# b4rtaz/distributed-llama

Hardware: AMD Instinct MI355X
Metric: decode tokens/s (Llama-3.1-8B Q40) (higher is better)
Workload: dtype f32-accum/int8-dot (Q40 weights, Q80 activations); 1 GPU; model=llama-3.1-8b, global_batch=1, seq_len=4096, prefill=32, parallelism=tp1, sync=q80, graph=True

## Files before the change

### dllama_amd/engine.py

```python

from __future__ import annotations

import time
from dataclasses import dataclass

import torch

from .tokenizer import Sampler


@dataclass
class GenStats:
    prefill_tokens: int = 0
    prefill_time: float = 0.0
    decode_tokens: int = 0
    decode_time: float = 0.0
    cached_tokens: int = 0

    @property
    def eval_tok_s(self) -> float:
        return self.prefill_tokens / self.prefill_time if self.prefill_time else 0.0

    @property
    def pred_tok_s(self) -> float:
# ... 100 lines not shown
            else:
                logits = self.decode_one(token)
                token = sampler.sample(logits)
            out.append(token)
            if on_token:
                on_token(token)
        self._sync_device()
        stats.decode_time = time.perf_counter() - t0
        stats.decode_tokens = len(out)
        return out, stats


class _Sequence:

    def __init__(self, prompt, max_tokens, sampler, on_token, stop_check):
        self.prompt = list(prompt)
        self.max_tokens = max_tokens
        self.sampler = sampler
        self.on_token = on_token
        self.stop_check = stop_check
        self.slot = None
        self.fed = 0
        self.pages = []
        self.registered = 0
        self.written = 0
        self.out: list[int] = []
        self.done = False
        self.stats = GenStats(prefill_tokens=len(self.prompt))
        self._t0 = None

    @property
    def tokens(self) -> list[int]:
        return self.out

    @property
    def prefilling(self) -> bool:
        return self.fed < len(self.prompt)


class BatchEngine:

    def __init__(self, model, tokenizer=None, n_batches: int = 32,
                 share_prefixes: bool = True):
        if not hasattr(model, "forward_rows"):
            raise ValueError("BatchEngine needs a model with forward_rows")
        self.model = model
        self.pool = None
        if getattr(model, "page_map", None) is not None:
            from .models.pages import PagePool
            self.pool = PagePool(model.kv_pages, model.page_size,
                                 share=share_prefixes)
            for slot in range(model.n_slots):
                model.clear_slot(slot)
        self.tokenizer = tokenizer
        self.n_batches = min(n_batches, getattr(model, "n_batches", n_batches))
        self.seq_len = model.cfg.seq_len
        self.free_slots = list(range(model.n_slots))
        self.waiting: list[_Sequence] = []
        self.running: list[_Sequence] = []
        self.last_step_rows: list[tuple] = []

    _coin = staticmethod(InferenceEngine._coin)

    def _on_device(self) -> bool:
        return (hasattr(self.model, "forward_rows_sample")
                and bool(getattr(self.model, "device_sampling", False)))

    def submit(self, prompt_tokens: list[int], max_tokens: int,
               sampler: Sampler | None = None, on_token=None,
               stop_check=None) -> _Sequence:
        if len(prompt_tokens) < 1:
            raise ValueError("empty prompt")
        if len(prompt_tokens) > self.seq_len:
            raise ValueError(
                f"prompt of {len(prompt_tokens)} tokens exceeds seq_len "
                f"{self.seq_len} (rebuild with a larger --max-seq-len / seq_len)")
        if self.pool is not None:
            need = self._pages_needed(len(prompt_tokens), max_tokens)
            if need > self.pool.n_pages:
                raise ValueError(
                    f"a request of {len(prompt_tokens)} prompt tokens and "
                    f"max_tokens {max_tokens} needs {need} KV pages, the pool "
                    f"has {self.pool.n_pages} (raise --kv-pages / kv_pages)")
        if sampler is None:
            sampler = Sampler(self.model.cfg.vocab_size, 0.0, 0.9, 12345)
        seq = _Sequence(prompt_tokens, max_tokens, sampler, on_token,
                        stop_check)
        self.waiting.append(seq)
        return seq

    @property
    def idle(self) -> bool:
        return not self.waiting and not self.running

    def _pages_needed(self, n_prompt: int, max_tokens: int) -> int:
        P = self.pool.page_size
        return -(-min(n_prompt + max_tokens, self.seq_len) // P)

    def _take_pages(self, seq: _Sequence) -> bool:
        pool = self.pool
        shared = pool.match(seq.prompt)
        need = self._pages_needed(len(seq.prompt), seq.max_tokens)
        new = pool.alloc(need - len(shared))
        if new is None:
            pool.release(shared)
            return False
# ... 128 lines not shown
```

### dllama_amd/models/hip_model.py

```python

from __future__ import annotations

import os

import numpy as np
import torch

from ..model_file import HIDDEN_ACT_GELU, ModelFile, ROPE_FALCON
from ..ops import hip_ops
from ..ops import reference as R
from ..ops.sampler import DeviceSampler
from ..parallel.comm import Comm, SingleComm
from ..quants import Q80, q40_to_planes
from .config import ModelConfig

QB = 32


class Linear:

    def __init__(self, qs: torch.Tensor, scales: torch.Tensor):
        self.qs = qs
        self.scales = scales
        self.d = qs.shape[-2]
# ... 71 lines not shown
        self.kv_pages = kv_pages
        self.page_size = page_size
        self.page_map = None
        self.page_table_sends = 0
        if kv_pages:
            from .rows import PageMap
            self.page_map = PageMap(n_slots, c.seq_len, kv_pages, page_size)
        self.comm = comm or SingleComm()
        self.tp_path = config.world > 1 or force_sync
        self.device = torch.device(device or "cuda")
        self.k = hip_ops()
        nb = 32
        if n_batches != 32:
            import warnings
            warnings.warn(
                f"HIP backend pins --n-batches to 32 (got {n_batches}): the "
                "prefill GEMM's MFMA fragment is 32 batch rows")
        self.n_batches = nb
        self.layers: list[dict] = []
        self.embedding = None
        self.final_norm = None
        self.wcls = None
        self._graph = None
        self._graph_pos = None
        self._graph_samples = False
        self._dev_sampler = None
        self.greedy_feedback = False
        self.skip_logits = False
        self._pf_graphs = {}
        self._pf_failed = False
        self.row_graphs = True
        self._row_graphs = {}
        self._row_graphs_failed = False
        self._rows_io = None
        self.kv_mul = c.n_heads0 // max(1, c.kv_dim0 // c.head_dim)
        self.rope_style = 1 if c.rope_type == ROPE_FALCON else 0
        self.fused_rope = self.rope_style == 0 and not c.is_qwen3
        self.row_bytes = c.dim + 2 * (c.dim // QB)
        self._read_options()
        self._alloc_buffers()

    def _read_options(self):
        env = os.environ

        def flag(name: str, default: str) -> bool:
            return env.get(name, default) == "1"

        self.attn_splits = int(env.get("DLLAMA_ATTN_SPLITS", "8"))
        self.fused_sync = flag("DLLAMA_FUSED_SYNC", "1")
        self.adaptive_thresh = int(env.get("DLLAMA_ADAPTIVE_SPLITS", "512"))
        if ("DLLAMA_ATTN_SPLITS" in env
                and "DLLAMA_ADAPTIVE_SPLITS" not in env):
            self.adaptive_thresh = 0
        self.fused_ffn = flag("DLLAMA_FUSED_FFN", "0")
        self.fused_moe = flag("DLLAMA_FUSED_MOE", "0")
        self.use_deferred = flag("DLLAMA_DEFERRED", "1")
        self.prefill_bf16 = flag("DLLAMA_PREFILL_BF16", "0")
        self.ksplit_resid = int(env.get("DLLAMA_KSPLIT_RESID", "0"))
        self.kv_f32 = flag("DLLAMA_KV_F32", "0")


    @classmethod
    def from_file(cls, m: ModelFile, config: ModelConfig, device=None,
                  comm: Comm | None = None, n_batches: int = 32,
                  force_sync: bool = False,
                  n_slots: int = 1, kv_pages: int = 0,
                  page_size: int = 64) -> "HipTransformer":
        from ..quants import Q40
        if m.header.weight_type != Q40:
            raise ValueError(
                "the MI355X HIP backend runs Q40 weights (the reference's "
                "shipped format); f32/q80 .m files run on the CPU backend "
                "(--gpu-index -1) or can be re-quantized with convert_hf.py")
        self = cls(config, device, comm, n_batches, force_sync, n_slots,
                   kv_pages, page_size)
        c, dev = config, self.device
        r, w = c.rank, c.world

        def lin(name, layer, d, n, expert=-1):
            e = m.entry(name, layer, expert)
            raw = m.slice_bytes(e, r, w)
            return Linear.from_blocks(raw, d, n, dev)

        def f32(name, layer=-1):
            return torch.from_numpy(np.array(m.f32(name, layer))).to(dev)

        def w13(l, expert=-1):
            return Linear.cat(lin("block_matmul_w1", l, c.ff_dim0, c.dim, expert),
                              lin("block_matmul_w3", l, c.ff_dim0, c.dim, expert))

        self.embedding = f32("embedding")
        self.final_norm = f32("final_norm")
        self.wcls = lin("final_matmul_logits", -1, c.vocab0, c.dim)
        for l in range(c.n_layers):
            lw = {
                "qkv": Linear.cat(lin("block_matmul_q", l, c.q_dim0, c.dim),
                                  lin("block_matmul_k", l, c.kv_dim0, c.dim),
                                  lin("block_matmul_v", l, c.kv_dim0, c.dim)),
                "wo": lin("block_matmul_wo", l, c.dim, c.q_dim0),
                "norm0": f32("block_norm_0", l),
                "norm1": f32("block_norm_1", l),
            }
            if c.is_moe:
                experts = range(c.n_experts)
                lw["gate"] = f32("block_moe_gate", l)
                lw["w13"] = Linear.stack([w13(l, e) for e in experts])
# ... 406 lines not shown
                           self.moe_idx[:ka], self.moe_out13, ka,
                           ssq_in=self.ssq[slot], eps=c.norm_eps)
        self._swiglu_q80(self.moe_out13, ka, self.moe_dq)
        k.q40_gemv_grouped(lw["w2"].qs, lw["w2"].scales, *self.moe_dq.triple(),
                           self.moe_idx[:ka], self.moe_y, 1)
        if self.tp_path:
            k.scale_merge_pack(self.moe_y, self.moe_wts,
                               self.sync_out[: self.row_bytes], 1, ka, c.dim)
            self._wire_exchange(1, self.ssq[slot + 1], wn)
        else:
            k.scale_merge_add_q(self.x[:1], self.moe_y, self.moe_wts,
                                self.ssq[slot + 1], wn, *self.xq.triple(),
                                1, ka)

    def _moe_ffn(self, B: int, NB: int, lw: dict, slot: int):
        c, k = self.cfg, self.k
        ka = c.n_active_experts
        S = NB * ka
        k.router_gemv(lw["gate"], self.t_norm, self.moe_router, NB)
        if c.ff_dim0 % 32 == 0 and ka <= 16 and self.fused_moe:
            wts, gate = self.moe_router[:NB], {"gate": True}
            k.q40_gemv_grouped_swiglu(lw["w13"].qs, lw["w13"].scales,
                                      *self.xq.triple(), *self.moe_dq.triple(),
                                      S, wts, ka)
            k.q40_gemv_grouped(lw["w2"].qs, lw["w2"].scales,
                               *self.moe_dq.triple(), self.moe_idx[:S],
                               self.moe_y, 1, router=wts, topk=ka, n_slots=S)
        else:
            wts, gate = self.moe_wts, {}
            k.moe_gate(self.moe_router[:NB], self.moe_idx, self.moe_wts, NB, ka)
            k.q40_gemv_grouped(lw["w13"].qs, lw["w13"].scales,
                               *self.xq.triple(), self.moe_idx[:S],
                               self.moe_out13, ka)
            self._swiglu_q80(self.moe_out13, S, self.moe_dq)
            k.q40_gemv_grouped(lw["w2"].qs, lw["w2"].scales,
                               *self.moe_dq.triple(), self.moe_idx[:S],
                               self.moe_y, 1)
        if not self.tp_path:
            k.scale_merge_add(self.x[:NB], self.moe_y, wts, self.ssq[slot],
                              NB, ka, **gate)
        else:
            k.scale_merge(self.partial[:NB], self.moe_y, wts, NB, ka, **gate)
            self._sync_partial(NB, slot)


    def forward(self, tokens: torch.Tensor, positions: torch.Tensor) -> torch.Tensor:
        B = tokens.shape[0]
        assert B <= self.n_batches
        p0 = self._first_position(positions, B)
        self.tokens[:B].copy_(tokens.to(self.device), non_blocking=True)
        if B == 1 and self._graph is not None:
            self._replay_decode(p0)
        else:
            g = None
            if B == self.n_batches and not self._pf_failed:
                g = (self._pf_graphs.get(self.skip_logits)
                     or self._capture_prefill_graph(self.skip_logits))
            self._step_at(B, p0, g)
        if self.tp_path:
            NBp = _pow2_batch(B)
            self.k.logits_concat(self.logits_full, self.logits_gather[NBp], B)
            return self.logits_full[:B]
        return self.logits0[:B]

    def _first_position(self, positions, B: int) -> int:
        self._rows_only()
        p0 = int(positions[0])
        if p0 + B > self.cfg.seq_len:
            raise ValueError(
                f"position {p0}+{B} exceeds seq_len {self.cfg.seq_len} "
                "(rebuild with a larger --max-seq-len / seq_len)")
        return p0

    def _step_at(self, B: int, p0: int, graph=None):
        self.pos.fill_(p0)
        self._graph_pos = None
        if graph is not None:
            graph.replay()
        else:
            self.forward_buffers(B)

    def _replay_decode(self, p0: int):
        sp = self._pick_splits(p0)
        if sp != self.attn_splits:
            self._set_attn_splits(sp)
        if p0 != self._graph_pos:
            self.pos.fill_(p0)
        self._graph.replay()
        self._graph_pos = p0 + 1


    def last_logits(self) -> torch.Tensor:
        if self.tp_path:
            return self.logits_gather[1].view(-1)[: self.cfg.vocab_size]
        return self.logits0[0]

    def _sampler(self) -> DeviceSampler:
        if self._dev_sampler is None:
            self._dev_sampler = DeviceSampler(
                self.cfg.vocab_size, self.device, params=self.sample_params,
                out=self.sample_out, k=self.k)
            self._step_host = torch.zeros(self.n_batches + 4,
                                          dtype=torch.int64).pin_memory()
        return self._dev_sampler

    def sample_row(self, row: torch.Tensor, coin, temperature: float,
                   topp: float):
        return self._sampler().sample(row, coin, temperature, topp)

    def forward_sample(self, tokens: torch.Tensor, positions: torch.Tensor,
                       coin, temperature: float, topp: float):
        assert tokens.shape[0] == 1
        p0 = self._first_position(positions, 1)
        smp, NB = self._sampler(), self.n_batches
        self._step_host[0] = int(tokens[0])
        smp.fill_params(self._step_host[NB:].view(torch.float64), coin,
                        temperature, topp)
        self._step_in.copy_(self._step_host, non_blocking=True)
        if self._graph is not None:
            self._replay_decode(p0)
            if not self._graph_samples:
                smp.launch(self.last_logits())
        else:
            self._step_at(1, p0)
            smp.launch(self.last_logits())
        return smp.read()


    def _rows_only(self):
        if self.page_map is not None:
            raise ValueError(
                "a paged model steps rows only (forward_rows); one sequence "
                "runs on the unpaged default")

    def _paged(self):
        if self.page_map is None:
            raise ValueError("the model has no paged KV cache (kv_pages=0)")
        return self.page_map

    def set_slot_pages(self, slot: int, pages, first: int = 0) -> None:
        self._paged().set_slot_pages(slot, pages, first)

    def clear_slot(self, slot: int) -> None:
        self._paged().clear_slot(slot)

    def _send_page_table(self):
        pm = self.page_map
        for slot in sorted(pm.dirty):
            self.page_table[slot].copy_(
                torch.tensor(pm.device_row(slot), dtype=torch.int32))
            self.page_table_sends += 1
        pm.dirty.clear()


    def _rows_buffers(self):
        if self._rows_io is None:
            NB, dev = self.n_batches, self.device
            self._rows_io = io = torch.zeros(6 * NB, dtype=torch.int64, device=dev)
            self.row_tokens = io[:NB]
            self.row_params = io[NB:5 * NB].view(torch.float64).view(NB, 4)
            self.rows = io[5 * NB:].view(torch.int32).view(NB, 2)
            if self.page_map is not None:
                self.row_addr = KVAddr("_paged", self.rows, self.page_table,
                                       self.page_size)
            else:
                self.row_addr = KVAddr("_rows", self.rows)
            self.rows_sample_out = torch.zeros(NB, 2, dtype=torch.int64,
                                               device=dev)
            self._rows_host = torch.zeros(6 * NB, dtype=torch.int64)
            if dev.type == "cuda":
                self._rows_host = self._rows_host.pin_memory()
            self._rows_copied = None
            self._rows_dev = []
            self._row_samplers = []
        return self._rows_io

# ... 20 lines not shown
            self.page_map.check(slots, positions)
            self._send_page_table()
            stride = self.page_map.pages_per_seq
        self._rows_buffers()
        if self._rows_copied is not None:
            self._rows_copied.synchronize()
        host = self._rows_host
        table = [(s * stride, p) for s, p in zip(slots, positions)]
        host[:NB] = 0
        host[:B] = torch.tensor(tokens, dtype=torch.int64)
        hp = host[NB:5 * NB].view(torch.float64).view(NB, 4)
        hp.zero_()
        if params is not None:
            hp[:B, :3] = torch.tensor(params, dtype=torch.float64)
        words = 5 * NB
        if self._rows_dev[:B] != table:
            ht = host[5 * NB:].view(torch.int32).view(NB, 2)
            ht.zero_()
            ht[:B] = torch.tensor(table, dtype=torch.int32)
            words = 6 * NB
            self._rows_dev = list(table)
        self._rows_io[:words].copy_(host[:words], non_blocking=True)
        if self.device.type == "cuda":
            self._rows_copied = torch.cuda.Event()
            self._rows_copied.record(torch.cuda.current_stream(self.device))
        return B, table, is_decode_step(slots)

    def _forward_rows_buffers(self, B: int):
        self._forward_explicit(B, self.row_addr)

    def _rows_step_and_sample(self, B: int):
        self._forward_rows_buffers(B)
        logits = self.rows_logits(B)
        for b in range(B):
            self._row_sampler(b).launch(logits[b])

    def _capture_rows_graph(self, B: int):
        try:
            for b in range(B):
                self._row_sampler(b)
            g = self._capture(lambda: self._rows_step_and_sample(B), warmups=2,
                              tail=lambda: self.k.rows_advance(self.rows, B))
            self._row_graphs[B] = g
            return g
        except Exception as e:
            import sys
            if self.comm.rank == 0:
                print(f"⚠️  row-step graph capture failed ({e}); "
                      "running eager (slower)", file=sys.stderr)
            self._row_graphs_failed = True
            return None

    def _run_rows(self, B: int, table, decode_only: bool, sample: bool):
        sp = self._pick_splits(max(p for _, p in table))
        if sp != self.attn_splits:
            self._set_attn_splits(sp)
        g = None
        if (decode_only and self.row_graphs and not self._row_graphs_failed
                and self.device.type == "cuda"):
            g = self._row_graphs.get(B) or self._capture_rows_graph(B)
        if g is not None:
            g.replay()
            self._rows_dev[:B] = [(base, p + 1) for base, p in table]
        elif sample:
            self._rows_step_and_sample(B)
        else:
            self._forward_rows_buffers(B)

    def forward_rows(self, tokens, slots, positions) -> torch.Tensor:
        B, table, decode_only = self._stage_rows(tokens, slots, positions)
        self._run_rows(B, table, decode_only, sample=False)
        return self.rows_logits(B)

    def forward_rows_sample(self, tokens, slots, positions, coins,
                            temperatures, topps) -> list:
        params = [(0.0 if c is None else float(c), float(t), float(p))
                  for c, t, p in zip(coins, temperatures, topps)]
        if len(params) != len(tokens):
            raise ValueError("one coin, temperature and topp per row")
        B, table, decode_only = self._stage_rows(tokens, slots, positions,
                                                 params)
        self._run_rows(B, table, decode_only, sample=True)
        return [None if status else token
                for token, status in self.rows_sample_out[:B].tolist()]


    def _pick_splits(self, pos: int) -> int:
        if not self.adaptive_thresh:
            return self.attn_splits
        if pos < self.adaptive_thresh:
            return 8
        return 16 if pos < 2048 else 32

    def _set_attn_splits(self, s: int):
        self.attn_splits = s
        self._alloc_attn_scratch()
        if self._graph is not None:
            pos_saved = int(self.pos.item())
            self.capture_decode_graph()
            self.pos.fill_(pos_saved)
            self._graph_pos = pos_saved
        self._pf_graphs.clear()
        self._row_graphs.clear()

    def _capture(self, body, warmups: int, tail=None):
        dev = self.device
        torch.cuda.synchronize(dev)
        s = torch.cuda.Stream(dev)
        s.wait_stream(torch.cuda.current_stream(dev))
        with torch.cuda.stream(s):
            for _ in range(warmups):
                body()
        torch.cuda.current_stream(dev).wait_stream(s)
        torch.cuda.synchronize(dev)
        g = torch.cuda.CUDAGraph()
        with torch.cuda.graph(g):
            body()
            if tail is not None:
                tail()
        return g

    def _capture_prefill_graph(self, skip_logits: bool):
        try:
            saved = self.skip_logits
            self.skip_logits = skip_logits
            g = self._capture(lambda: self.forward_buffers(self.n_batches),
                              warmups=1)
            self.skip_logits = saved
            self._pf_graphs[skip_logits] = g
            return g
        except Exception:
            self._pf_failed = True
            self.skip_logits = skip_logits
            return None

    def capture_decode_graph(self):
        self._rows_only()
        sample = bool(self.device_sampling)
        if sample:
            self._sampler()

        def step():
            self.forward_buffers(1)
            if sample:
                self._sampler().launch(self.last_logits())

        self._graph = self._capture(
            step, warmups=2, tail=lambda: self.k.pos_inc(self.pos, 1))
# ... 3 lines not shown
```

### dllama_amd/ops/csrc/attn.hip

```cpp

#include "dllama_common.h"

struct SeqRows {
    static constexpr bool kPaged = false;
    const int *pos;
    __device__ int position(int b) const { return pos[0] + b; }
    __device__ int64_t cache_base(int) const { return 0; }
    __device__ int64_t cache_row(int, int t) const { return t; }
};
struct TableRows {
    static constexpr bool kPaged = false;
    const int *rows;
    __device__ int position(int b) const { return rows[2 * b + 1]; }
    __device__ int64_t cache_base(int b) const { return rows[2 * b]; }
    __device__ int64_t cache_row(int b, int t) const {
        return (int64_t)rows[2 * b] + t;
    }
};
struct PagedRows {
    static constexpr bool kPaged = true;
    const int *rows;
    const int *pages;
    int shift;
    __device__ int position(int b) const { return rows[2 * b + 1]; }
    __device__ int64_t cache_base(int) const { return 0; }
    __device__ const int *seq_pages(int b) const { return pages + rows[2 * b]; }
    __device__ int64_t cache_row(int b, int t) const {
        return ((int64_t)seq_pages(b)[t >> shift] << shift)
             + (t & ((1 << shift) - 1));
    }
};

template <int VEC, typename KVT, bool FUSE = false, typename ROWS = SeqRows>
__global__ void k_attn_split(const float *__restrict__ q, int q_ld,
                             const KVT *__restrict__ kc_all,
                             const KVT *__restrict__ vc_all,
                             const ROWS rows,
                             int n_heads0, int kv_mul, int kv_dim0, float scale,
                             float *__restrict__ ml_scratch,
                             float *__restrict__ o_scratch,
                             int *__restrict__ counter,
                             float *__restrict__ y,
                             int8_t *__restrict__ zq,
                             float *__restrict__ zs,
                             float *__restrict__ zbs) {
    (void)counter; (void)y; (void)zq; (void)zs; (void)zbs;
    const int h0 = blockIdx.x;
    const int b = blockIdx.y;
    const int sp = blockIdx.z;
    const int S = gridDim.z;
    const int hd = VEC * WAVE;
    const int plen = rows.position(b) + 1;
    const KVT *kc = kc_all + rows.cache_base(b) * kv_dim0;
    const KVT *vc = vc_all + rows.cache_base(b) * kv_dim0;
    const int wave = ROWS::kPaged
        ? __builtin_amdgcn_readfirstlane(threadIdx.x / WAVE)
        : threadIdx.x / WAVE;
    const int lane = threadIdx.x % WAVE;
    const int kv_off = (h0 / kv_mul) * hd;

    const int VEC16 = VEC * 4;
    const int lane16 = lane & 15;
    const int group = lane >> 4;

    float qreg[VEC16];
    #pragma unroll
    for (int v = 0; v < VEC16; v++)
        qreg[v] = q[(int64_t)b * q_ld + h0 * hd + lane16 * VEC16 + v] * scale;

    float m = -1e30f, l = 0.0f, o[VEC];
    #pragma unroll
    for (int v = 0; v < VEC; v++) o[v] = 0.0f;

    const int stride = 16 * S;
    [[maybe_unused]] int pg[4];
    [[maybe_unused]] const int *seq_pages = nullptr;
    [[maybe_unused]] int pshift = 0;
    if constexpr (ROWS::kPaged) {
        seq_pages = rows.seq_pages(b);
        pshift = rows.shift;
        #pragma unroll
        for (int u = 0; u < 4; u++) {
            const int t = (sp * 4 + wave) * 4 + u * stride;
            pg[u] = t < plen ? seq_pages[t >> pshift] : 0;
        }
    }
    for (int tb0 = (sp * 4 + wave) * 4; tb0 < plen; tb0 += 4 * stride) {
        [[maybe_unused]] int64_t rb[4];
        if constexpr (ROWS::kPaged) {
            #pragma unroll
            for (int u = 0; u < 4; u++) {
                const int t = tb0 + u * stride;
                rb[u] = ((int64_t)pg[u] << pshift) + (t & ((1 << pshift) - 1));
            }
            #pragma unroll
            for (int u = 0; u < 4; u++) {
                const int t = tb0 + 4 * stride + u * stride;
                pg[u] = t < plen ? seq_pages[t >> pshift] : 0;
            }
// ... 14 lines not shown
        }
        float s16[16];
        float mn = m;
        #pragma unroll
        for (int u = 0; u < 4; u++) {
            #pragma unroll
            for (int gg = 0; gg < 4; gg++) {
                float v = __shfl(su[u], gg * 16, WAVE);
                if (tb0 + u * stride + gg >= plen) v = -1e30f;
                s16[4 * u + gg] = v;
                mn = fmaxf(mn, v);
            }
        }
        const float f = __expf(m - mn);
        float w16[16];
        float lsum = 0.0f;
        #pragma unroll
        for (int i = 0; i < 16; i++) {
            w16[i] = __expf(s16[i] - mn);
            lsum += w16[i];
        }
        l = l * f + lsum;
        #pragma unroll
        for (int v = 0; v < VEC; v++) o[v] *= f;
        #pragma unroll
        for (int u = 0; u < 4; u++) {
            #pragma unroll
            for (int gg = 0; gg < 4; gg++) {
                const int t = tb0 + u * stride + gg;
                if (t >= plen) continue;
                const int64_t vr = ROWS::kPaged ? rb[u] + gg : (int64_t)t;
                const KVT *vrow = vc + vr * kv_dim0 + kv_off + lane * VEC;
                #pragma unroll
                for (int v = 0; v < VEC; v++)
                    o[v] = fmaf(w16[4 * u + gg], kv_f(vrow[v]), o[v]);
            }
        }
        m = mn;
    }

    __shared__ float sm[4], sl[4];
    __shared__ float so[4][VEC * WAVE];
    if (lane == 0) { sm[wave] = m; sl[wave] = l; }
    __syncthreads();
    const float M = fmaxf(fmaxf(sm[0], sm[1]), fmaxf(sm[2], sm[3]));
    const float fw = __expf(m - M);
    #pragma unroll
    for (int v = 0; v < VEC; v++) so[wave][lane * VEC + v] = o[v] * fw;
    __syncthreads();
    const int64_t slot = ((int64_t)b * n_heads0 + h0) * S + sp;
    if (wave == 0) {
        const float L = sl[0] * __expf(sm[0] - M) + sl[1] * __expf(sm[1] - M)
                      + sl[2] * __expf(sm[2] - M) + sl[3] * __expf(sm[3] - M);
        if constexpr (FUSE) {
            const float invL = 1.0f / L;
            float vv[VEC];
            #pragma unroll
            for (int v = 0; v < VEC; v++) {
                const int i = lane * VEC + v;
                vv[v] = (so[0][i] + so[1][i] + so[2][i] + so[3][i]) * invL;
            }
            if constexpr (VEC == 2) {
                const float amax = group16_reduce_max(fmaxf(fabsf(vv[0]), fabsf(vv[1])));
                const float dd = amax / 127.0f;
                const float qinv = dd > 0.0f ? 1.0f / dd : 0.0f;
                const float q0 = rintf(vv[0] * qinv), q1 = rintf(vv[1] * qinv);
                const int64_t obase = ((int64_t)b * n_heads0 + h0) * hd + lane * 2;
                zq[obase] = (int8_t)q0;
                zq[obase + 1] = (int8_t)q1;
                const float bsum = group16_reduce_sum(q0 + q1);
                if ((lane & 15) == 0) {
                    const int blk = (h0 * hd + lane * 2) / QB;
                    zs[(int64_t)b * (n_heads0 * hd / QB) + blk] = dd;
                    zbs[(int64_t)b * (n_heads0 * hd / QB) + blk] = bsum;
                }
            } else {
                const Q80Lane c = q80_quant_group32(vv[0]);
                zq[((int64_t)b * n_heads0 + h0) * hd + lane] = (int8_t)c.qf;
                const float bsum = group32_reduce_sum(c.qf);
                if ((lane & 31) == 0) {
                    const int blk = (h0 * hd + lane) / QB;
                    zs[(int64_t)b * (n_heads0 * hd / QB) + blk] = c.d;
                    zbs[(int64_t)b * (n_heads0 * hd / QB) + blk] = bsum;
                }
            }
        } else {
            if (lane == 0) {
                ml_scratch[slot * 2] = M;
                ml_scratch[slot * 2 + 1] = L;
            }
            #pragma unroll
            for (int v = 0; v < VEC; v++) {
                const int i = lane * VEC + v;
                o_scratch[slot * hd + i] = so[0][i] + so[1][i] + so[2][i] + so[3][i];
            }
        }
    }

}

template <int VEC, typename KVT>
__global__ void k_attn_split_gqa(const float *__restrict__ q, int q_ld,
                                 const KVT *__restrict__ kc,
                                 const KVT *__restrict__ vc,
                                 const int *__restrict__ pos,
                                 int n_heads0, int kv_mul, int kv_dim0,
                                 float scale,
                                 float *__restrict__ ml_scratch,
                                 float *__restrict__ o_scratch) {
    const int kvh = blockIdx.x;
    const int b = blockIdx.y;
    const int sp = blockIdx.z;
    const int S = gridDim.z;
    const int hd = VEC * WAVE;
    const int plen = pos[0] + b + 1;
    const int wave = threadIdx.x / WAVE;
    const int lane = threadIdx.x % WAVE;
    const int h0 = kvh * kv_mul + wave;
    const int kv_off = kvh * hd;
    const int VEC16 = VEC * 4;
    const int lane16 = lane & 15;
    const int group = lane >> 4;

    float qreg[VEC16];
    #pragma unroll
    for (int v = 0; v < VEC16; v++)
        qreg[v] = q[(int64_t)b * q_ld + h0 * hd + lane16 * VEC16 + v] * scale;

    float m = -1e30f, l = 0.0f, o[VEC];
    #pragma unroll
    for (int v = 0; v < VEC; v++) o[v] = 0.0f;

    for (int tb0 = sp * 16; tb0 < plen; tb0 += 16 * S) {
        float su[4];
        #pragma unroll
        for (int u = 0; u < 4; u++) {
            const int tg = tb0 + u * 4 + group;
            float partial = 0.0f;
            if (tg < plen) {
                const KVT *krow = kc + (int64_t)tg * kv_dim0 + kv_off + lane16 * VEC16;
                #pragma unroll
                for (int v = 0; v < VEC16; v++)
                    partial = fmaf(qreg[v], kv_f(krow[v]), partial);
            }
            su[u] = group16_reduce_sum(partial);
        }
        float s16[16];
        float mn = m;
        #pragma unroll
        for (int u = 0; u < 4; u++) {
            #pragma unroll
            for (int gg = 0; gg < 4; gg++) {
// ... 267 lines not shown

void kv_append(torch::Tensor k, torch::Tensor v, torch::Tensor kc,
               torch::Tensor vc, torch::Tensor pos) {
    CHECK_CUDA(k);
    const int B = k.size(0);
    const int kv_dim0 = k.size(1);
    const dim3 grid(ceil_div(kv_dim0, 256), B);
    with_kv_ptrs(kc, vc, [&](auto *kcp, auto *vcp) {
        using KVT = std::remove_pointer_t<decltype(kcp)>;
        hipLaunchKernelGGL(k_kv_append<KVT>, grid, dim3(256), 0, cur_stream(),
                           k.data_ptr<float>(), v.data_ptr<float>(), kcp, vcp,
                           pos.data_ptr<int>(), kv_dim0);
    });
}

static TableRows table_rows(const torch::Tensor &rows, int64_t batch) {
    CHECK_CUDA(rows);
    TORCH_CHECK(rows.scalar_type() == at::kInt && rows.dim() == 2
                && rows.size(1) == 2 && rows.is_contiguous()
                && rows.size(0) >= batch,
                "row table must be a contiguous int32 [>= batch, 2]");
    return TableRows{rows.data_ptr<int>()};
}

static PagedRows paged_rows(const torch::Tensor &rows,
                            const torch::Tensor &page_table, int64_t page_size,
                            int64_t batch, const torch::Tensor &kc) {
    const TableRows t = table_rows(rows, batch);
    CHECK_CUDA(page_table);
    TORCH_CHECK(page_table.scalar_type() == at::kInt && page_table.dim() == 2
                && page_table.is_contiguous() && page_table.numel() > 0
                && page_table.device() == kc.device()
                && rows.device() == kc.device(),
                "page table must be a contiguous int32 [n_slots, "
                "pages_per_seq] on the cache's device");
    TORCH_CHECK(page_size >= 4 && page_size <= 256
                && (page_size & (page_size - 1)) == 0,
                "page_size must be a power of two in 4..256 (got ",
                page_size, ")");
    TORCH_CHECK(kc.size(0) % page_size == 0,
                "a paged cache holds whole pages: ", kc.size(0),
                " rows, page_size ", page_size);
    int shift = 0;
    while ((int64_t(1) << shift) < page_size) shift++;
    return PagedRows{t.rows, page_table.data_ptr<int>(), shift};
}

template <typename ROWS>
static void attn_launch(torch::Tensor &q, int64_t q_ld, torch::Tensor &kc,
                        torch::Tensor &vc, torch::Tensor &y, ROWS rows,
                        int64_t batch, int64_t n_heads0, int64_t kv_mul,
                        int64_t head_dim, int64_t splits,
                        torch::Tensor &ml_scratch, torch::Tensor &o_scratch,
                        int *counter, bool allow_variants,
                        c10::optional<torch::Tensor> &zq,
                        c10::optional<torch::Tensor> &zs,
                        c10::optional<torch::Tensor> &zbs) {
    CHECK_CUDA(q);
    const int kv_dim0 = kc.size(1);
    const float scale = 1.0f / sqrtf((float)head_dim);
    const dim3 grid(n_heads0, batch, splits);
    const dim3 cgrid(n_heads0, batch);
    const bool quant = zq.has_value();
    float *yp = quant ? nullptr : y.data_ptr<float>();
    int8_t *zqp = quant ? zq->data_ptr<int8_t>() : nullptr;
    float *zsp = quant ? zs->data_ptr<float>() : nullptr;
    float *zbsp = quant ? zbs->data_ptr<float>() : nullptr;
    static const bool env_gqa =
        std::getenv("DLLAMA_GQA_ATTN") && atoi(std::getenv("DLLAMA_GQA_ATTN")) == 1;
    const bool gqa = allow_variants && env_gqa && kv_mul > 1 && kv_mul <= 8
        && n_heads0 % kv_mul == 0 && splits > 1;
    const bool fused = allow_variants && !gqa && splits == 1 && quant;
    with_head_vec(head_dim, [&](auto vec_const) {
        constexpr int V = decltype(vec_const)::value;
        with_kv_ptrs(kc, vc, [&](auto *kcp, auto *vcp) {
            using KVT = std::remove_pointer_t<decltype(kcp)>;
            auto split = [&](auto fuse_const) {
                constexpr bool FUSE = decltype(fuse_const)::value;
                hipLaunchKernelGGL((k_attn_split<V, KVT, FUSE, ROWS>), grid,
                                   dim3(256), 0,
                                   cur_stream(), q.data_ptr<float>(), (int)q_ld,
                                   kcp, vcp, rows,
                                   (int)n_heads0, (int)kv_mul, kv_dim0, scale,
                                   ml_scratch.data_ptr<float>(),
                                   o_scratch.data_ptr<float>(),
                                   counter, nullptr,
                                   FUSE ? zqp : nullptr, FUSE ? zsp : nullptr,
                                   FUSE ? zbsp : nullptr);
            };
            if constexpr (std::is_same_v<ROWS, SeqRows>) {
                if (gqa) {
                    hipLaunchKernelGGL((k_attn_split_gqa<V, KVT>),
                                       dim3(n_heads0 / kv_mul, batch, splits),
                                       dim3(kv_mul * WAVE), 0,
                                       cur_stream(), q.data_ptr<float>(), (int)q_ld,
                                       kcp, vcp, rows.pos, (int)n_heads0,
                                       (int)kv_mul, kv_dim0, scale,
                                       ml_scratch.data_ptr<float>(),
                                       o_scratch.data_ptr<float>());
                    return;
                }
                if (fused) {
                    split(std::true_type{});
                    return;
                }
            }
            split(std::false_type{});
        });
        if (fused) return;
        auto combine = [&](auto quant_const) {
            hipLaunchKernelGGL((k_attn_combine<V, decltype(quant_const)::value>),
                               cgrid, dim3(V * WAVE), 0, cur_stream(),
                               ml_scratch.data_ptr<float>(),
                               o_scratch.data_ptr<float>(), yp, zqp, zsp, zbsp,
                               (int)n_heads0, (int)splits);
        };
        if (quant) combine(std::true_type{});
        else combine(std::false_type{});
    });
}

void attn(torch::Tensor q, int64_t q_ld, torch::Tensor kc, torch::Tensor vc,
          torch::Tensor y, torch::Tensor pos, int64_t batch, int64_t n_heads0,
          int64_t kv_mul, int64_t head_dim, int64_t splits,
          torch::Tensor ml_scratch, torch::Tensor o_scratch, torch::Tensor counter,
          c10::optional<torch::Tensor> zq = c10::nullopt,
          c10::optional<torch::Tensor> zs = c10::nullopt,
          c10::optional<torch::Tensor> zbs = c10::nullopt) {
    attn_launch(q, q_ld, kc, vc, y, SeqRows{pos.data_ptr<int>()}, batch,
                n_heads0, kv_mul, head_dim, splits, ml_scratch, o_scratch,
                counter.data_ptr<int>(), true, zq, zs, zbs);
}

void attn_rows(torch::Tensor q, int64_t q_ld, torch::Tensor kc, torch::Tensor vc,
               torch::Tensor y, torch::Tensor rows, int64_t batch,
               int64_t n_heads0, int64_t kv_mul, int64_t head_dim,
               int64_t splits, torch::Tensor ml_scratch, torch::Tensor o_scratch,
               c10::optional<torch::Tensor> zq = c10::nullopt,
               c10::optional<torch::Tensor> zs = c10::nullopt,
               c10::optional<torch::Tensor> zbs = c10::nullopt) {
    attn_launch(q, q_ld, kc, vc, y, table_rows(rows, batch), batch, n_heads0,
                kv_mul, head_dim, splits, ml_scratch, o_scratch, nullptr,
                false, zq, zs, zbs);
}

void attn_paged(torch::Tensor q, int64_t q_ld, torch::Tensor kc, torch::Tensor vc,
                torch::Tensor y, torch::Tensor rows, torch::Tensor page_table,
                int64_t page_size, int64_t batch, int64_t n_heads0,
                int64_t kv_mul, int64_t head_dim, int64_t splits,
                torch::Tensor ml_scratch, torch::Tensor o_scratch,
                c10::optional<torch::Tensor> zq = c10::nullopt,
                c10::optional<torch::Tensor> zs = c10::nullopt,
                c10::optional<torch::Tensor> zbs = c10::nullopt) {
    attn_launch(q, q_ld, kc, vc, y,
                paged_rows(rows, page_table, page_size, batch, kc), batch,
                n_heads0, kv_mul, head_dim, splits, ml_scratch, o_scratch,
                nullptr, false, zq, zs, zbs);
}

template <typename ROWS>
static void rope_kv_launch(torch::Tensor &qkv, int64_t ld, int64_t q_dim0,
                           int64_t kv_dim0, torch::Tensor &cache, ROWS rows,
                           torch::Tensor &kc, torch::Tensor &vc,
                           int64_t head_dim, int64_t style, int64_t batch) {
    CHECK_CUDA(qkv);
    const int total = (int)(q_dim0 / 2 + kv_dim0 / 2 + kv_dim0 / 4);
    const dim3 grid(ceil_div(total, 256), batch);
    with_kv_ptrs(kc, vc, [&](auto *kcp, auto *vcp) {
        using KVT = std::remove_pointer_t<decltype(kcp)>;
        auto *kern = style == 0 ? k_rope_kv<0, KVT, ROWS> : k_rope_kv<1, KVT, ROWS>;
        hipLaunchKernelGGL(kern, grid, dim3(256), 0, cur_stream(),
                           qkv.data_ptr<float>(), (int)ld, (int)q_dim0, (int)kv_dim0,
                           cache.data_ptr<float>(), rows,
                           kcp, vcp, (int)head_dim);
    });
}

void rope_kv(torch::Tensor qkv, int64_t ld, int64_t q_dim0, int64_t kv_dim0,
             torch::Tensor cache, torch::Tensor pos, torch::Tensor kc,
             torch::Tensor vc, int64_t head_dim, int64_t style, int64_t batch) {
    rope_kv_launch(qkv, ld, q_dim0, kv_dim0, cache,
                   SeqRows{pos.data_ptr<int>()}, kc, vc, head_dim, style, batch);
}

void rope_kv_rows(torch::Tensor qkv, int64_t ld, int64_t q_dim0, int64_t kv_dim0,
                  torch::Tensor cache, torch::Tensor rows, torch::Tensor kc,
                  torch::Tensor vc, int64_t head_dim, int64_t style,
                  int64_t batch) {
    rope_kv_launch(qkv, ld, q_dim0, kv_dim0, cache, table_rows(rows, batch),
                   kc, vc, head_dim, style, batch);
}

void rope_kv_paged(torch::Tensor qkv, int64_t ld, int64_t q_dim0, int64_t kv_dim0,
                   torch::Tensor cache, torch::Tensor rows,
                   torch::Tensor page_table, int64_t page_size,
                   torch::Tensor kc, torch::Tensor vc, int64_t head_dim,
                   int64_t style, int64_t batch) {
    rope_kv_launch(qkv, ld, q_dim0, kv_dim0, cache,
                   paged_rows(rows, page_table, page_size, batch, kc), kc, vc,
                   head_dim, style, batch);
}

template <typename ROWS>
static void rope_kv_qknorm_launch(torch::Tensor &qkv, int64_t ld, int64_t q_dim0,
                                  int64_t kv_dim0, torch::Tensor &cache,
                                  ROWS rows, torch::Tensor &kc,
                                  torch::Tensor &vc, int64_t head_dim,
                                  torch::Tensor &wq, torch::Tensor &wk,
                                  double eps, int64_t batch) {
    CHECK_CUDA(qkv);
// ... 82 lines not shown
```

Measured before the change: 491.0 tokens/s.

## Add single-block wide attention kernel with fused Q80 output for short contexts

```diff
diff --git a/dllama_amd/engine.py b/dllama_amd/engine.py
--- a/dllama_amd/engine.py
+++ b/dllama_amd/engine.py
@@ -176,6 +176,8 @@
                                  share=share_prefixes)
             for slot in range(model.n_slots):
                 model.clear_slot(slot)
+        if hasattr(model, "set_wide_rows"):
+            model.set_wide_rows()
         self.tokenizer = tokenizer
         self.n_batches = min(n_batches, getattr(model, "n_batches", n_batches))
         self.seq_len = model.cfg.seq_len
diff --git a/dllama_amd/models/hip_model.py b/dllama_amd/models/hip_model.py
--- a/dllama_amd/models/hip_model.py
+++ b/dllama_amd/models/hip_model.py
@@ -147,6 +147,9 @@
         if ("DLLAMA_ATTN_SPLITS" in env
                 and "DLLAMA_ADAPTIVE_SPLITS" not in env):
             self.adaptive_thresh = 0
+        self.wide_thresh = int(env.get("DLLAMA_ATTN_WIDE", "256"))
+        self.wide_rows = flag("DLLAMA_ATTN_WIDE_ROWS", "0")
+        self._splits_above = self.attn_splits if self.attn_splits != 1 else 8
         self.fused_ffn = flag("DLLAMA_FUSED_FFN", "0")
         self.fused_moe = flag("DLLAMA_FUSED_MOE", "0")
         self.use_deferred = flag("DLLAMA_DEFERRED", "1")
@@ -659,6 +662,8 @@
         if B == 1 and self._graph is not None:
             self._replay_decode(p0)
         else:
+            self._follow_wide_tier(
+                p0 + B - 1, emit_q80=not (B >= 8 and self.prefill_bf16))
             g = None
             if B == self.n_batches and not self._pf_failed:
                 g = (self._pf_graphs.get(self.skip_logits)
@@ -686,6 +691,11 @@
             graph.replay()
         else:
             self.forward_buffers(B)
+
+    def _follow_wide_tier(self, last_pos: int, emit_q80: bool):
+        wide = emit_q80 and self._pick_splits(last_pos) == 1
+        if wide != (self.attn_splits == 1):
+            self._set_attn_splits(1 if wide else self._splits_above)
 
     def _replay_decode(self, p0: int):
         sp = self._pick_splits(p0)
@@ -729,6 +739,7 @@
             if not self._graph_samples:
                 smp.launch(self.last_logits())
         else:
+            self._follow_wide_tier(p0, emit_q80=True)
             self._step_at(1, p0)
             smp.launch(self.last_logits())
         return smp.read()
@@ -855,7 +866,7 @@
             return None
 
     def _run_rows(self, B: int, table, decode_only: bool, sample: bool):
-        sp = self._pick_splits(max(p for _, p in table))
+        sp = self._pick_splits(max(p for _, p in table), rows=True)
         if sp != self.attn_splits:
             self._set_attn_splits(sp)
         g = None
@@ -888,15 +899,23 @@
                 for token, status in self.rows_sample_out[:B].tolist()]
 
 
-    def _pick_splits(self, pos: int) -> int:
+    def _pick_splits(self, pos: int, rows: bool = False) -> int:
         if not self.adaptive_thresh:
             return self.attn_splits
+        if ((self.wide_rows or not rows)
+                and pos < min(self.wide_thresh, self.adaptive_thresh)):
+            return 1
         if pos < self.adaptive_thresh:
             return 8
         return 16 if pos < 2048 else 32
 
+    def set_wide_rows(self, on: bool = True):
+        self.wide_rows = on
+
     def _set_attn_splits(self, s: int):
         self.attn_splits = s
+        if s != 1:
+            self._splits_above = s
         self._alloc_attn_scratch()
         if self._graph is not None:
             pos_saved = int(self.pos.item())
diff --git a/dllama_amd/ops/csrc/attn.hip b/dllama_amd/ops/csrc/attn.hip
--- a/dllama_amd/ops/csrc/attn.hip
+++ b/dllama_amd/ops/csrc/attn.hip
@@ -31,20 +31,14 @@
     }
 };
 
-template <int VEC, typename KVT, bool FUSE = false, typename ROWS = SeqRows>
+template <int VEC, typename KVT, typename ROWS = SeqRows>
 __global__ void k_attn_split(const float *__restrict__ q, int q_ld,
                              const KVT *__restrict__ kc_all,
                              const KVT *__restrict__ vc_all,
                              const ROWS rows,
                              int n_heads0, int kv_mul, int kv_dim0, float scale,
                              float *__restrict__ ml_scratch,
-                             float *__restrict__ o_scratch,
-                             int *__restrict__ counter,
-                             float *__restrict__ y,
-                             int8_t *__restrict__ zq,
-                             float *__restrict__ zs,
-                             float *__restrict__ zbs) {
-    (void)counter; (void)y; (void)zq; (void)zs; (void)zbs;
+                             float *__restrict__ o_scratch) {
     const int h0 = blockIdx.x;
     const int b = blockIdx.y;
     const int sp = blockIdx.z;
@@ -165,52 +159,183 @@
     if (wave == 0) {
         const float L = sl[0] * __expf(sm[0] - M) + sl[1] * __expf(sm[1] - M)
                       + sl[2] * __expf(sm[2] - M) + sl[3] * __expf(sm[3] - M);
-        if constexpr (FUSE) {
-            const float invL = 1.0f / L;
-            float vv[VEC];
+        if (lane == 0) {
+            ml_scratch[slot * 2] = M;
+            ml_scratch[slot * 2 + 1] = L;
+        }
+        #pragma unroll
+        for (int v = 0; v < VEC; v++) {
+            const int i = lane * VEC + v;
+            o_scratch[slot * hd + i] = so[0][i] + so[1][i] + so[2][i] + so[3][i];
+        }
+    }
+}
+
+
+template <typename T, int N>
+struct alignas(sizeof(T) * N) KVPack { T e[N]; };
+
+template <int BYTES> struct UIntOfSize;
+template <> struct UIntOfSize<2> { using type = unsigned short; };
+template <> struct UIntOfSize<4> { using type = unsigned int; };
+template <> struct UIntOfSize<8> { using type = unsigned long long; };
+template <typename P>
+__device__ __forceinline__ P load_in_order(const P *p) {
+    using U = typename UIntOfSize<sizeof(P)>::type;
+    const U u = __hip_atomic_load(reinterpret_cast<const U *>(p),
+                                  __ATOMIC_RELAXED,
+                                  __HIP_MEMORY_SCOPE_WAVEFRONT);
+    P r;
+    __builtin_memcpy(&r, &u, sizeof(P));
+    return r;
+}
+
+#define ATTN_WIDE_ROWS(X) \
+    X(0, 0) X(0, 1) X(0, 2) X(0, 3) X(1, 0) X(1, 1) X(1, 2) X(1, 3) \
+    X(2, 0) X(2, 1) X(2, 2) X(2, 3) X(3, 0) X(3, 1) X(3, 2) X(3, 3)
+
+template <int VEC, typename KVT, typename ROWS>
+__global__ void __launch_bounds__(1024)
+k_attn_wide(const float *__restrict__ q, int q_ld,
+            const KVT *__restrict__ kc_all,
+            const KVT *__restrict__ vc_all,
+            const ROWS rows,
+            int n_heads0, int kv_mul, int kv_dim0, float scale,
+            int8_t *__restrict__ zq,
+            float *__restrict__ zs,
+            float *__restrict__ zbs) {
+    constexpr int NW = 16;
+    constexpr int hd = VEC * WAVE;
+    constexpr int VEC16 = VEC * 4;
+    using KPack = KVPack<KVT, VEC16>;
+    using VPack = KVPack<KVT, VEC>;
+    const int h0 = blockIdx.x;
+    const int b = blockIdx.y;
+    const int plen = rows.position(b) + 1;
+    const KVT *kc = kc_all + rows.cache_base(b) * kv_dim0;
+    const KVT *vc = vc_all + rows.cache_base(b) * kv_dim0;
+    const int wave = __builtin_amdgcn_readfirstlane(threadIdx.x / WAVE);
+    const int lane = threadIdx.x % WAVE;
+    const int kv_off = (h0 / kv_mul) * hd;
+    const int lane16 = lane & 15;
+    const int group = lane >> 4;
+
+    float qreg[VEC16];
+    #pragma unroll
+    for (int v = 0; v < VEC16; v++)
+        qreg[v] = q[(int64_t)b * q_ld + h0 * hd + lane16 * VEC16 + v];
+
+    float m = -1e30f, l = 0.0f, o[VEC];
+    #pragma unroll
+    for (int v = 0; v < VEC; v++) o[v] = 0.0f;
+
+    const int tlast = plen - 1;
+    [[maybe_unused]] int pg[4];
+    if constexpr (ROWS::kPaged) {
+        #pragma unroll
+        for (int u = 0; u < 4; u++)
+            pg[u] = rows.seq_pages(b)[min(wave * 16 + u * 4, tlast & ~3)
+                                      >> rows.shift];
+    }
+
+    for (int tb = wave * 16; tb < plen; tb += 16 * NW) {
+        int trow[4];
+        int64_t roff[4];
+        #pragma unroll
+        for (int u = 0; u < 4; u++) {
+            trow[u] = min(tb + u * 4, tlast & ~3);
+            int64_t r = trow[u];
+            if constexpr (ROWS::kPaged)
+                r = ((int64_t)pg[u] << rows.shift)
+                  + (trow[u] & ((1 << rows.shift) - 1));
+            roff[u] = r * kv_dim0 + kv_off;
+        }
+        KPack kk[4];
+        #pragma unroll
+        for (int u = 0; u < 4; u++) {
+            const int g = min(trow[u] + group, tlast) - trow[u];
+            kk[u] = *reinterpret_cast<const KPack *>(
+                kc + roff[u] + (g * kv_dim0 + lane16 * VEC16));
+        }
+        #define X(u, g) \
+            const VPack v##u##g = load_in_order(reinterpret_cast<const VPack *>( \
+                vc + roff[u] + (min(trow[u] + g, tlast) - trow[u]) * kv_dim0 \
+                + lane * VEC));
+        ATTN_WIDE_ROWS(X)
+        #undef X
+        __builtin_amdgcn_sched_barrier(0);
+
+        float s16[16];
+        float mn = m;
+        #pragma unroll
+        for (int u = 0; u < 4; u++) {
+            float partial = 0.0f;
             #pragma unroll
-            for (int v = 0; v < VEC; v++) {
-                const int i = lane * VEC + v;
-                vv[v] = (so[0][i] + so[1][i] + so[2][i] + so[3][i]) * invL;
-            }
-            if constexpr (VEC == 2) {
-                const float amax = group16_reduce_max(fmaxf(fabsf(vv[0]), fabsf(vv[1])));
-                const float dd = amax / 127.0f;
-                const float qinv = dd > 0.0f ? 1.0f / dd : 0.0f;
-                const float q0 = rintf(vv[0] * qinv), q1 = rintf(vv[1] * qinv);
-                const int64_t obase = ((int64_t)b * n_heads0 + h0) * hd + lane * 2;
-                zq[obase] = (int8_t)q0;
-                zq[obase + 1] = (int8_t)q1;
-                const float bsum = group16_reduce_sum(q0 + q1);
-                if ((lane & 15) == 0) {
-                    const int blk = (h0 * hd + lane * 2) / QB;
-                    zs[(int64_t)b * (n_heads0 * hd / QB) + blk] = dd;
-                    zbs[(int64_t)b * (n_heads0 * hd / QB) + blk] = bsum;
-                }
-            } else {
-                const Q80Lane c = q80_quant_group32(vv[0]);
-                zq[((int64_t)b * n_heads0 + h0) * hd + lane] = (int8_t)c.qf;
-                const float bsum = group32_reduce_sum(c.qf);
-                if ((lane & 31) == 0) {
-                    const int blk = (h0 * hd + lane) / QB;
-                    zs[(int64_t)b * (n_heads0 * hd / QB) + blk] = c.d;
-                    zbs[(int64_t)b * (n_heads0 * hd / QB) + blk] = bsum;
-                }
-            }
-        } else {
-            if (lane == 0) {
-                ml_scratch[slot * 2] = M;
-                ml_scratch[slot * 2 + 1] = L;
-            }
+            for (int v = 0; v < VEC16; v++)
+                partial = fmaf(qreg[v], kv_f(kk[u].e[v]), partial);
+            const float su = group16_reduce_sum(partial) * scale;
             #pragma unroll
-            for (int v = 0; v < VEC; v++) {
-                const int i = lane * VEC + v;
-                o_scratch[slot * hd + i] = so[0][i] + so[1][i] + so[2][i] + so[3][i];
-            }
-        }
-    }
-
-}
+            for (int gg = 0; gg < 4; gg++) {
+                float v = __shfl(su, gg * 16, WAVE);
+                if (tb + u * 4 + gg >= plen) v = -1e30f;
+                s16[4 * u + gg] = v;
+                mn = fmaxf(mn, v);
+            }
+        }
+        const float f = __expf(m - mn);
+        float w16[16];
+        float lsum = 0.0f;
+        #pragma unroll
+        for (int i = 0; i < 16; i++) {
+            w16[i] = __expf(s16[i] - mn);
+            lsum += w16[i];
+        }
+        l = l * f + lsum;
+        #pragma unroll
+        for (int v = 0; v < VEC; v++) o[v] *= f;
+        #define X(u, g) \
+            _Pragma("unroll") \
+            for (int v = 0; v < VEC; v++) \
+                o[v] = fmaf(w16[4 * u + g], kv_f(v##u##g.e[v]), o[v]);
+        ATTN_WIDE_ROWS(X)
+        #undef X
+        m = mn;
+        if constexpr (ROWS::kPaged) {
+            #pragma unroll
+            for (int u = 0; u < 4; u++)
+                pg[u] = rows.seq_pages(b)[min(tb + 16 * NW + u * 4, tlast & ~3)
+                                          >> rows.shift];
+        }
+    }
+
+    __shared__ float sm[NW], sl[NW];
+    __shared__ float so[NW][hd];
+    if (lane == 0) { sm[wave] = m; sl[wave] = l; }
+    #pragma unroll
+    for (int v = 0; v < VEC; v++) so[wave][lane * VEC + v] = o[v];
+    __syncthreads();
+    if (threadIdx.x >= hd) return;
+    const int i = threadIdx.x;
+    float M = -1e30f;
+    #pragma unroll
+    for (int w = 0; w < NW; w++) M = fmaxf(M, sm[w]);
+    float L = 0.0f, acc = 0.0f;
+    #pragma unroll
+    for (int w = 0; w < NW; w++) {
+        const float fw = __expf(sm[w] - M);
+        L = fmaf(sl[w], fw, L);
+        acc = fmaf(so[w][i], fw, acc);
+    }
+    const Q80Lane c = q80_quant_group32(acc * (1.0f / L));
+    zq[((int64_t)b * n_heads0 + h0) * hd + i] = (int8_t)c.qf;
+    const float bsum = group32_reduce_sum(c.qf);
+    if ((i & 31) == 0) {
+        const int blk = (h0 * hd + i) / QB;
+        zs[(int64_t)b * (n_heads0 * hd / QB) + blk] = c.d;
+        zbs[(int64_t)b * (n_heads0 * hd / QB) + blk] = bsum;
+    }
+}
+#undef ATTN_WIDE_ROWS
 
 template <int VEC, typename KVT>
 __global__ void k_attn_split_gqa(const float *__restrict__ q, int q_ld,
@@ -584,7 +709,6 @@
                         int64_t batch, int64_t n_heads0, int64_t kv_mul,
                         int64_t head_dim, int64_t splits,
                         torch::Tensor &ml_scratch, torch::Tensor &o_scratch,
-                        int *counter, bool allow_variants,
                         c10::optional<torch::Tensor> &zq,
                         c10::optional<torch::Tensor> &zs,
                         c10::optional<torch::Tensor> &zbs) {
@@ -600,26 +724,21 @@
     float *zbsp = quant ? zbs->data_ptr<float>() : nullptr;
     static const bool env_gqa =
         std::getenv("DLLAMA_GQA_ATTN") && atoi(std::getenv("DLLAMA_GQA_ATTN")) == 1;
-    const bool gqa = allow_variants && env_gqa && kv_mul > 1 && kv_mul <= 8
-        && n_heads0 % kv_mul == 0 && splits > 1;
-    const bool fused = allow_variants && !gqa && splits == 1 && quant;
+    const bool gqa = std::is_same_v<ROWS, SeqRows> && env_gqa && kv_mul > 1
+        && kv_mul <= 8 && n_heads0 % kv_mul == 0 && splits > 1;
+    const bool wide = splits == 1 && quant;
     with_head_vec(head_dim, [&](auto vec_const) {
         constexpr int V = decltype(vec_const)::value;
         with_kv_ptrs(kc, vc, [&](auto *kcp, auto *vcp) {
             using KVT = std::remove_pointer_t<decltype(kcp)>;
-            auto split = [&](auto fuse_const) {
-                constexpr bool FUSE = decltype(fuse_const)::value;
-                hipLaunchKernelGGL((k_attn_split<V, KVT, FUSE, ROWS>), grid,
-                                   dim3(256), 0,
-                                   cur_stream(), q.data_ptr<float>(), (int)q_ld,
-                                   kcp, vcp, rows,
-                                   (int)n_heads0, (int)kv_mul, kv_dim0, scale,
-                                   ml_scratch.data_ptr<float>(),
-                                   o_scratch.data_ptr<float>(),
-                                   counter, nullptr,
-                                   FUSE ? zqp : nullptr, FUSE ? zsp : nullptr,
-                                   FUSE ? zbsp : nullptr);
-            };
+            if (wide) {
+                hipLaunchKernelGGL((k_attn_wide<V, KVT, ROWS>), cgrid,
+                                   dim3(1024), 0, cur_stream(),
+                                   q.data_ptr<float>(), (int)q_ld, kcp, vcp,
+                                   rows, (int)n_heads0, (int)kv_mul, kv_dim0,
+                                   scale, zqp, zsp, zbsp);
+                return;
+            }
             if constexpr (std::is_same_v<ROWS, SeqRows>) {
                 if (gqa) {
                     hipLaunchKernelGGL((k_attn_split_gqa<V, KVT>),
@@ -632,14 +751,15 @@
                                        o_scratch.data_ptr<float>());
                     return;
                 }
-                if (fused) {
-                    split(std::true_type{});
-                    return;
-                }
-            }
-            split(std::false_type{});
+            }
+            hipLaunchKernelGGL((k_attn_split<V, KVT, ROWS>), grid, dim3(256),
+                               0, cur_stream(), q.data_ptr<float>(), (int)q_ld,
+                               kcp, vcp, rows,
+                               (int)n_heads0, (int)kv_mul, kv_dim0, scale,
+                               ml_scratch.data_ptr<float>(),
+                               o_scratch.data_ptr<float>());
         });
-        if (fused) return;
+        if (wide) return;
         auto combine = [&](auto quant_const) {
             hipLaunchKernelGGL((k_attn_combine<V, decltype(quant_const)::value>),
                                cgrid, dim3(V * WAVE), 0, cur_stream(),
@@ -655,13 +775,14 @@
 void attn(torch::Tensor q, int64_t q_ld, torch::Tensor kc, torch::Tensor vc,
           torch::Tensor y, torch::Tensor pos, int64_t batch, int64_t n_heads0,
           int64_t kv_mul, int64_t head_dim, int64_t splits,
-          torch::Tensor ml_scratch, torch::Tensor o_scratch, torch::Tensor counter,
+          torch::Tensor ml_scratch, torch::Tensor o_scratch,
+          torch::Tensor ,
           c10::optional<torch::Tensor> zq = c10::nullopt,
           c10::optional<torch::Tensor> zs = c10::nullopt,
           c10::optional<torch::Tensor> zbs = c10::nullopt) {
     attn_launch(q, q_ld, kc, vc, y, SeqRows{pos.data_ptr<int>()}, batch,
                 n_heads0, kv_mul, head_dim, splits, ml_scratch, o_scratch,
-                counter.data_ptr<int>(), true, zq, zs, zbs);
+                zq, zs, zbs);
 }
 
 void attn_rows(torch::Tensor q, int64_t q_ld, torch::Tensor kc, torch::Tensor vc,
@@ -672,8 +793,7 @@
                c10::optional<torch::Tensor> zs = c10::nullopt,
                c10::optional<torch::Tensor> zbs = c10::nullopt) {
     attn_launch(q, q_ld, kc, vc, y, table_rows(rows, batch), batch, n_heads0,
-                kv_mul, head_dim, splits, ml_scratch, o_scratch, nullptr,
-                false, zq, zs, zbs);
+                kv_mul, head_dim, splits, ml_scratch, o_scratch, zq, zs, zbs);
 }
 
 void attn_paged(torch::Tensor q, int64_t q_ld, torch::Tensor kc, torch::Tensor vc,
@@ -687,7 +807,7 @@
     attn_launch(q, q_ld, kc, vc, y,
                 paged_rows(rows, page_table, page_size, batch, kc), batch,
                 n_heads0, kv_mul, head_dim, splits, ml_scratch, o_scratch,
-                nullptr, false, zq, zs, zbs);
+                zq, zs, zbs);
 }
 
 template <typename ROWS>
```

Result: faster. 574.0 tokens/s, median of 6 (+16.9%).
